# k2-fsa/Flow2GAN

Hardware: AMD Instinct MI355X
Metric: audio-seconds/sec (train step, G+D fwd/bwd) mel_24k_base (higher is better)
Workload: dtype f32 (fp32-class products on the bf16 matrix pipe for the long reductions and the direct MRD convs: every fp32 operand as three bf16 pieces = 24 significand bits, the six v_mfma_f32_32x32x16_bf16 products with i + j <= 2 per fp32 product, fp32 accumulate, error <= 2^-23 per product; short reductions ; 1 GPU; mel_24k_base GAN stage-2 train step: D-step + G-step, each on its own batch (MPD+MRD+FM+multi-scale mel), fwd+bwd+grad all-reduce, no optimizer (metric is fwd/bwd); per_gpu_batch=64, gan=gan_multi_scale_mel_recon, parallelism=dp1, optimizer=none

## Files before the change

flow2gan_amd/csrc/conv2ch.hip:

```cpp
#include <stdlib.h>

#include "common.h"

namespace {

typedef float f32x16 __attribute__((ext_vector_type(16)));

constexpr int KH = 3, KW = 9, NTAP = KH * KW, CO = 32;
constexpr int TW = 32;
constexpr int PW = TW + KW - 1;
constexpr int FTH = 8;
constexpr int FPH = FTH + KH - 1;

__device__ __forceinline__ void stage_patch(float* plane, const f2g_conv2ch_desc& d,
                                            const float* xs, int h0, int w0, int rows, int tid,
                                            int nthreads) {
  for (int i = tid; i < rows * PW; i += nthreads) {
    const int r = i / PW, c = i - r * PW;
    const int h = h0 - 1 + r, w = w0 - 4 + c;
    float2 v = make_float2(0.f, 0.f);
    if (h >= 0 && h < d.H && w >= 0 && w < d.W)
      v = *reinterpret_cast<const float2*>(xs + (long long)h * d.x_line + (long long)w * 2);
    plane[i] = v.x;
    plane[rows * PW + i] = v.y;
  }
}

__global__ __launch_bounds__(256) void conv2ch_fwd_kernel(const f2g_conv2ch_desc d) {
  __shared__ float plane[2 * FPH * PW];
  const int tid = threadIdx.x, lane = tid & 63, wave = tid >> 6;
  const int li = lane & 31, h = lane >> 5;
  const int tiles_w = (d.W + TW - 1) / TW;
  const int tw = blockIdx.x % tiles_w, th = blockIdx.x / tiles_w;
  const int s = blockIdx.y;
  const int h0 = th * FTH, w0 = tw * TW;
  stage_patch(plane, d, d.x + (long long)s * d.x_seq, h0, w0, FPH, tid, 256);
  float bw[NTAP];
#pragma unroll
  for (int t = 0; t < NTAP; ++t) bw[t] = d.w[li * (NTAP * 2) + t * 2 + h];
  const float bias = d.bias ? d.bias[li] : 0.f;
  __syncthreads();
  const float* pl = plane + h * (FPH * PW);
#pragma unroll
  for (int rr = 0; rr < FTH / 4; ++rr) {
    const int row = wave + 4 * rr;
    if (h0 + row >= d.H) break;
    f32x16 acc;
#pragma unroll
    for (int e = 0; e < 16; ++e) acc[e] = bias;
#pragma unroll
    for (int t = 0; t < NTAP; ++t) {
      const int dh = t / KW, j = t - dh * KW;
      const float a = pl[(row + dh) * PW + li + j];
      acc = __builtin_amdgcn_mfma_f32_32x32x2f32(a, bw[t], acc, 0, 0, 0);
    }
    float* yrow = d.y + ((long long)s * d.H + h0 + row) * (long long)d.W * CO;
#pragma unroll
    for (int e = 0; e < 16; ++e) {
      const int col = w0 + (e & 3) + 8 * (e >> 2) + 4 * h;
      if (col < d.W) {
        float v = acc[e];
        if (d.lrelu_slope != 0.f) v = v > 0.f ? v : d.lrelu_slope * v;
        yrow[(long long)col * CO + li] = v;
      }
    }
  }
}

__global__ __launch_bounds__(256) void conv2ch_fwd_p_kernel(const f2g_conv2ch_desc d) {
  __shared__ float plane[2][2 * FPH * PW];
  const int tid = threadIdx.x, lane = tid & 63, wave = tid >> 6;
  const int li = lane & 31, h = lane >> 5;
  const int s = blockIdx.y, w0 = blockIdx.x * TW;
  const float* xs = d.x + (long long)s * d.x_seq;
  float bw[NTAP];
#pragma unroll
  for (int t = 0; t < NTAP; ++t) bw[t] = d.w[li * (NTAP * 2) + t * 2 + h];
  const float bias = d.bias ? d.bias[li] : 0.f;
  constexpr int NP = (FPH * PW + 255) / 256;
  int pr[NP], pc[NP];
#pragma unroll
  for (int q = 0; q < NP; ++q) {
    const int i = tid + 256 * q;
    pr[q] = i / PW;
    pc[q] = i - pr[q] * PW;
  }
  auto load_patch = [&](int h0, float2 (&v)[NP]) {
#pragma unroll
    for (int q = 0; q < NP; ++q) {
      const int hh = h0 - 1 + pr[q], ww = w0 - 4 + pc[q];
      const bool ok = tid + 256 * q < FPH * PW && hh >= 0 && hh < d.H && ww >= 0 && ww < d.W;
      v[q] = ok ? *reinterpret_cast<const float2*>(xs + (long long)hh * d.x_line + (long long)ww * 2)
                : make_float2(0.f, 0.f);
    }
  };
  auto store_patch = [&](float* pl, const float2 (&v)[NP]) {
#pragma unroll
    for (int q = 0; q < NP; ++q) {
      const int i = tid + 256 * q;
      if (i < FPH * PW) {
        pl[i] = v[q].x;
        pl[FPH * PW + i] = v[q].y;
      }
    }
  };
  {
    float2 v[NP];
    load_patch(0, v);
    store_patch(plane[0], v);
  }
  __syncthreads();
  int cur = 0;
  for (int h0 = 0; h0 < d.H; h0 += FTH) {
    const bool more = h0 + FTH < d.H;
    float2 nv[NP];
    load_patch(more ? h0 + FTH : h0, nv);
    const float* pl = plane[cur] + h * (FPH * PW);
#pragma unroll
    for (int rr = 0; rr < FTH / 4; ++rr) {
      const int row = wave + 4 * rr;
      if (h0 + row < d.H) {
        f32x16 acc;
#pragma unroll
        for (int e = 0; e < 16; ++e) acc[e] = bias;
#pragma unroll
        for (int t = 0; t < NTAP; ++t) {
          const int dh = t / KW, j = t - dh * KW;
          acc = __builtin_amdgcn_mfma_f32_32x32x2f32(pl[(row + dh) * PW + li + j], bw[t], acc, 0, 0, 0);
        }
        float* yrow = d.y + ((long long)s * d.H + h0 + row) * (long long)d.W * CO;
#pragma unroll
        for (int e = 0; e < 16; ++e) {
          const int col = w0 + (e & 3) + 8 * (e >> 2) + 4 * h;
          if (col < d.W) {
            float v = acc[e];
            if (d.lrelu_slope != 0.f) v = v > 0.f ? v : d.lrelu_slope * v;
            yrow[(long long)col * CO + li] = v;
          }
        }
      }
    }
    if (more) store_patch(plane[cur ^ 1], nv);
    __syncthreads();
    cur ^= 1;
  }
}

__global__ __launch_bounds__(256) void conv2ch_wgrad_p_kernel(const f2g_conv2ch_desc d, int tiles_h,
                                                              int tiles_w, int tiles_per_block) {
  __shared__ float plane[2 * FPH * PW];
  __shared__ __attribute__((aligned(16))) float gt[FTH * TW * CO];
  const int tid = threadIdx.x, lane = tid & 63, wave = tid >> 6;
  const int li = lane & 31, h = lane >> 5;
  const int ntiles = d.S * tiles_h * tiles_w;
  int boff[2];
  bool bok[2];
#pragma unroll
  for (int nt = 0; nt < 2; ++nt) {
    const int n = li + 32 * nt;
    bok[nt] = n < NTAP * 2;
    const int t = bok[nt] ? n >> 1 : 0, ci = n & 1;
    const int dh = t / KW, j = t - dh * KW;
    boff[nt] = ci * (FPH * PW) + dh * PW + j;
  }
  f32x16 acc[2];
#pragma unroll
  for (int nt = 0; nt < 2; ++nt)
#pragma unroll
    for (int e = 0; e < 16; ++e) acc[nt][e] = 0.f;
  constexpr int NP = (FPH * PW + 255) / 256, NG = FTH * TW * (CO / 4) / 256;
  const int c4 = tid & 7;
  auto load_tile = [&](int ti, float2 (&pv)[NP], float4 (&gv)[NG]) {
    const int s = ti / (tiles_h * tiles_w), rem = ti - s * (tiles_h * tiles_w);
    const int th = rem / tiles_w, tw = rem - th * tiles_w;
    const int h0 = th * FTH, w0 = tw * TW;
    const float* xs = d.x + (long long)s * d.x_seq;
#pragma unroll
    for (int q = 0; q < NP; ++q) {
      const int i = tid + 256 * q, r = i / PW, c = i - r * PW;
      const int hh = h0 - 1 + r, ww = w0 - 4 + c;
      const bool ok = i < FPH * PW && hh >= 0 && hh < d.H && ww >= 0 && ww < d.W;
      pv[q] = ok ? *reinterpret_cast<const float2*>(xs + (long long)hh * d.x_line + (long long)ww * 2)
                 : make_float2(0.f, 0.f);
    }
#pragma unroll
    for (int q = 0; q < NG; ++q) {
      const int px = (tid >> 3) + 32 * q;
      const int row = px / TW, col = px - row * TW;
      const bool ok = h0 + row < d.H && w0 + col < d.W;
      gv[q] = ok ? *reinterpret_cast<const float4*>(d.y + (((long long)s * d.H + h0 + row) * (long long)d.W + w0 + col) * CO + c4 * 4)
                 : make_float4(0.f, 0.f, 0.f, 0.f);
    }
  };
  auto store_tile = [&](const float2 (&pv)[NP], const float4 (&gv)[NG]) {
#pragma unroll
    for (int q = 0; q < NP; ++q) {
      const int i = tid + 256 * q;
      if (i < FPH * PW) {
        plane[i] = pv[q].x;
        plane[FPH * PW + i] = pv[q].y;
      }
    }
#pragma unroll
    for (int q = 0; q < NG; ++q)
      *reinterpret_cast<float4*>(gt + ((tid >> 3) + 32 * q) * CO + c4 * 4) = gv[q];
  };
  const int t0 = blockIdx.x * tiles_per_block;
  int tend = t0 + tiles_per_block;
  if (tend > ntiles) tend = ntiles;
  if (t0 >= tend) return;
  {
    float2 pv[NP];
    float4 gv[NG];
    load_tile(t0, pv, gv);
    store_tile(pv, gv);
  }
  __syncthreads();
  for (int ti = t0; ti < tend; ++ti) {
    const bool more = ti + 1 < tend;
    float2 pv[NP];
    float4 gv[NG];
    load_tile(more ? ti + 1 : ti, pv, gv);
#pragma unroll
    for (int rr = 0; rr < FTH / 4; ++rr) {
      const int row = wave + 4 * rr;
      const float* grow = gt + row * TW * CO + li;
#pragma unroll
      for (int st = 0; st < TW / 2; ++st) {
        const int col = 2 * st + h;
        const float a = grow[col * CO];
        const float b0 = bok[0] ? plane[boff[0] + row * PW + col] : 0.f;
        const float b1 = bok[1] ? plane[boff[1] + row * PW + col] : 0.f;
        acc[0] = __builtin_amdgcn_mfma_f32_32x32x2f32(a, b0, acc[0], 0, 0, 0);
        acc[1] = __builtin_amdgcn_mfma_f32_32x32x2f32(a, b1, acc[1], 0, 0, 0);
      }
    }
    __syncthreads();
    if (more) store_tile(pv, gv);
    __syncthreads();
  }
#pragma unroll
  for (int nt = 0; nt < 2; ++nt) {
    const int n = li + 32 * nt;
    if (n >= NTAP * 2) continue;
#pragma unroll
    for (int e = 0; e < 16; ++e) {
      const int co = (e & 3) + 8 * (e >> 2) + 4 * h;
      atomicAdd(d.gw + co * (NTAP * 2) + n, acc[nt][e]);
    }
  }
}

constexpr int DTH = 8;
constexpr int DPH = DTH + KH - 1;
constexpr int GP = 36;

__global__ __launch_bounds__(256) void conv2ch_dgrad_kernel(const f2g_conv2ch_desc d) {
  extern __shared__ __attribute__((aligned(16))) float gp[];
  const int tid = threadIdx.x;
  const int tiles_w = (d.W + TW - 1) / TW;
  const int tw = blockIdx.x % tiles_w, th = blockIdx.x / tiles_w;
  const int s = blockIdx.y;
  const int h0 = th * DTH, w0 = tw * TW;
  const float* gs = d.y + (long long)s * d.H * d.W * CO;
  for (int i = tid; i < DPH * PW * (CO / 4); i += 256) {
    const int c4 = i & 7, px = i >> 3;
    const int r = px / PW, c = px - r * PW;
    const int hh = h0 - 1 + r, ww = w0 - 4 + c;
    float4 v = make_float4(0.f, 0.f, 0.f, 0.f);
    if (hh >= 0 && hh < d.H && ww >= 0 && ww < d.W)
      v = *reinterpret_cast<const float4*>(gs + ((long long)hh * d.W + ww) * CO + c4 * 4);
    *reinterpret_cast<float4*>(gp + px * GP + c4 * 4) = v;
  }
  __syncthreads();
  const int pw = tid & 31, ph = tid >> 5;
  float a0 = 0.f, a1 = 0.f;
#pragma unroll
  for (int dh = 0; dh < KH; ++dh)
#pragma unroll
    for (int j = 0; j < KW; ++j) {
      const float* g0 = gp + ((ph + 2 - dh) * PW + pw + 8 - j) * GP;
      const float* wt = d.wt + (dh * KW + j) * (2 * CO);
#pragma unroll
      for (int c4 = 0; c4 < CO / 4; ++c4) {
        const float4 gv = *reinterpret_cast<const float4*>(g0 + c4 * 4);
        a0 += gv.x * wt[c4 * 4] + gv.y * wt[c4 * 4 + 1] + gv.z * wt[c4 * 4 + 2] + gv.w * wt[c4 * 4 + 3];
        a1 += gv.x * wt[CO + c4 * 4] + gv.y * wt[CO + c4 * 4 + 1] + gv.z * wt[CO + c4 * 4 + 2] +
              gv.w * wt[CO + c4 * 4 + 3];
      }
    }
  const int hh = h0 + ph, ww = w0 + pw;
  if (hh < d.H && ww < d.W) {
    float* o = d.gx + (long long)s * d.gx_seq + (long long)hh * d.gx_line + (long long)ww * 2;
    *reinterpret_cast<float2*>(o) = make_float2(a0, a1);
  }
}

constexpr int QTH = 8, QTW = 32;
constexpr int QPH = QTH + 2, QPW = QTW + 2;

__device__ __forceinline__ void stage32(float* patch, const float* xs, int H, int W, int h0, int w0,
                                        int tid) {
  for (int i = tid; i < QPH * QPW * (CO / 4); i += 256) {
    const int c4 = i & 7, px = i >> 3;
    const int r = px / QPW, c = px - r * QPW;
    const int hh = h0 - 1 + r, ww = w0 - 1 + c;
    float4 v = make_float4(0.f, 0.f, 0.f, 0.f);
    if (hh >= 0 && hh < H && ww >= 0 && ww < W)
      v = *reinterpret_cast<const float4*>(xs + ((long long)hh * W + ww) * CO + c4 * 4);
    *reinterpret_cast<float4*>(patch + px * GP + c4 * 4) = v;
  }
}

__global__ __launch_bounds__(256) void convpost_fwd_kernel(const f2g_conv2ch_desc d) {
  extern __shared__ __attribute__((aligned(16))) float patch[];
  const int tid = threadIdx.x;
  const int tiles_w = (d.W + QTW - 1) / QTW;
  const int tw = blockIdx.x % tiles_w, th = blockIdx.x / tiles_w;
  const int s = blockIdx.y;
  const int h0 = th * QTH, w0 = tw * QTW;
  __shared__ __attribute__((aligned(16))) float wl[9 * CO];
  for (int i = tid; i < 9 * CO; i += 256) wl[i] = d.w[i];
  stage32(patch, d.x + (long long)s * d.H * d.W * CO, d.H, d.W, h0, w0, tid);
  __syncthreads();
  const int pw = tid & 31, ph = tid >> 5;
  float a0 = 0.f, a1 = 0.f;
#pragma unroll 1
  for (int t = 0; t < 9; ++t) {
    const float* x0 = patch + ((ph + t / 3) * QPW + pw + t % 3) * GP;
    const float* wt = wl + t * CO;
#pragma unroll
    for (int c4 = 0; c4 < CO / 4; c4 += 2) {
      const float4 u = *reinterpret_cast<const float4*>(x0 + c4 * 4);
      const float4 v = *reinterpret_cast<const float4*>(x0 + c4 * 4 + 4);
      const float4 wu = *reinterpret_cast<const float4*>(wt + c4 * 4);
      const float4 wv = *reinterpret_cast<const float4*>(wt + c4 * 4 + 4);
      a0 += u.x * wu.x + u.y * wu.y + u.z * wu.z + u.w * wu.w;
      a1 += v.x * wv.x + v.y * wv.y + v.z * wv.z + v.w * wv.w;
    }
  }
  const int hh = h0 + ph, ww = w0 + pw;
  if (hh < d.H && ww < d.W)
    d.y[((long long)s * d.H + hh) * d.W + ww] = a0 + a1 + (d.bias ? d.bias[0] : 0.f);
}

__global__ __launch_bounds__(256) void convpost_wgrad_kernel(const f2g_conv2ch_desc d, int px_per_block) {
  __shared__ float red[32][9 * CO + 1];
  const int tid = threadIdx.x, c4 = tid & 7, pg = tid >> 3;
  const long long npx = (long long)d.S * d.H * d.W;
  float4 acc[9];
#pragma unroll
  for (int t = 0; t < 9; ++t) acc[t] = make_float4(0.f, 0.f, 0.f, 0.f);
  const long long p0 = (long long)blockIdx.x * px_per_block;
  const long long pend = p0 + px_per_block < npx ? p0 + px_per_block : npx;
  constexpr int U = 4;
  for (long long p = p0 + pg; p < pend; p += 32 * U) {
    float4 v[U];
    float gn[U][9];
#pragma unroll
    for (int u = 0; u < U; ++u) {
      const long long q = p + 32 * u;
      const bool on = q < pend;
      const long long qq = on ? q : p;
      v[u] = *reinterpret_cast<const float4*>(d.x + qq * CO + c4 * 4);
      const int w = (int)(qq % d.W);
      const int h = (int)((qq / d.W) % d.H);
#pragma unroll
      for (int t = 0; t < 9; ++t) {
        const int oh = h - (t / 3 - 1), ow = w - (t % 3 - 1);
        const bool ok = on && oh >= 0 && oh < d.H && ow >= 0 && ow < d.W;
        gn[u][t] = ok ? d.y[qq - (long long)(t / 3 - 1) * d.W - (t % 3 - 1)] : 0.f;
      }
    }
#pragma unroll
    for (int u = 0; u < U; ++u)
#pragma unroll
      for (int t = 0; t < 9; ++t) {
        acc[t].x += gn[u][t] * v[u].x; acc[t].y += gn[u][t] * v[u].y;
        acc[t].z += gn[u][t] * v[u].z; acc[t].w += gn[u][t] * v[u].w;
      }
  }
#pragma unroll
  for (int t = 0; t < 9; ++t) {
    red[pg][t * CO + c4 * 4 + 0] = acc[t].x; red[pg][t * CO + c4 * 4 + 1] = acc[t].y;
    red[pg][t * CO + c4 * 4 + 2] = acc[t].z; red[pg][t * CO + c4 * 4 + 3] = acc[t].w;
  }
  __syncthreads();
  for (int k = tid; k < 9 * CO; k += 256) {
    float s = 0.f;
#pragma unroll 8
    for (int g2 = 0; g2 < 32; ++g2) s += red[g2][k];
    atomicAdd(d.gw + k, s);
  }
}

__global__ __launch_bounds__(256) void convpost_dgrad_kernel(const f2g_conv2ch_desc d) {
  const long long npx = (long long)d.S * d.H * d.W;
  const int c4 = threadIdx.x & 7;
  float4 wv[9];
#pragma unroll
  for (int t = 0; t < 9; ++t) wv[t] = *reinterpret_cast<const float4*>(d.w + t * CO + c4 * 4);
  for (long long i = (long long)blockIdx.x * 32 + (threadIdx.x >> 3); i < npx;
       i += (long long)gridDim.x * 32) {
    const int ww = (int)(i % d.W);
    const long long q = i / d.W;
    const int hh = (int)(q % d.H);
    float4 a = make_float4(0.f, 0.f, 0.f, 0.f);
#pragma unroll
    for (int t = 0; t < 9; ++t) {
      const int sh = hh + 1 - t / 3, sw = ww + 1 - t % 3;
      if (sh >= 0 && sh < d.H && sw >= 0 && sw < d.W) {
        const float gv = d.y[i + (long long)(1 - t / 3) * d.W + (1 - t % 3)];
        a.x += gv * wv[t].x; a.y += gv * wv[t].y; a.z += gv * wv[t].z; a.w += gv * wv[t].w;
      }
    }
    *reinterpret_cast<float4*>(d.gx + i * CO + c4 * 4) = a;
  }
}

}

#define ST ((hipStream_t)stream)

static bool conv2ch_ok(const f2g_conv2ch_desc* d) {
  return d && d->S > 0 && d->H > 0 && d->W > 0;
}

extern "C" int f2g_conv2ch_fwd(const f2g_conv2ch_desc* d, f2g_stream_t stream) {
  if (!d || !d->x || !d->w || !d->y || (d->x_line & 1) || (d->x_seq & 1)) return F2G_EINVAL;
  if (!conv2ch_ok(d)) return F2G_OK;
  if ((long long)((d->W + TW - 1) / TW) * d->S >= 256) {
    hipLaunchKernelGGL(conv2ch_fwd_p_kernel, dim3((d->W + TW - 1) / TW, d->S), dim3(256), 0, ST, *d);
    return f2g_check_launch();
  }
  const int tiles = ((d->H + FTH - 1) / FTH) * ((d->W + TW - 1) / TW);
  hipLaunchKernelGGL(conv2ch_fwd_kernel, dim3(tiles, d->S), dim3(256), 0, ST, *d);
  return f2g_check_launch();
}

extern "C" int f2g_conv2ch_wgrad(const f2g_conv2ch_desc* d, f2g_stream_t stream) {
  if (!d || !d->x || !d->y || !d->gw || (d->x_line & 1) || (d->x_seq & 1)) return F2G_EINVAL;
  if (((uintptr_t)d->y) & 15) return F2G_EINVAL;
  if (!conv2ch_ok(d)) return F2G_OK;
  const int tiles_h = (d->H + FTH - 1) / FTH, tiles_w = (d->W + TW - 1) / TW;
  const int ntiles = d->S * tiles_h * tiles_w;
  int per = (ntiles + 511) / 512;
  if (per < 1) per = 1;
  hipLaunchKernelGGL(conv2ch_wgrad_p_kernel, dim3((ntiles + per - 1) / per), dim3(256), 0, ST, *d,
                     tiles_h, tiles_w, per);
  return f2g_check_launch();
}

extern "C" int f2g_conv2ch_dgrad(const f2g_conv2ch_desc* d, f2g_stream_t stream) {
  if (!d || !d->y || !d->wt || !d->gx || (d->gx_line & 1) || (d->gx_seq & 1)) return F2G_EINVAL;
  if ((((uintptr_t)d->y) & 15) || (((uintptr_t)d->gx) & 7)) return F2G_EINVAL;
  if (!conv2ch_ok(d)) return F2G_OK;
  const size_t smem = (size_t)DPH * PW * GP * sizeof(float);
  static bool attr_done = false;
  if (!attr_done) {
    (void)hipFuncSetAttribute(reinterpret_cast<const void*>(conv2ch_dgrad_kernel),
                              hipFuncAttributeMaxDynamicSharedMemorySize, (int)smem);
    attr_done = true;
  }
  const int tiles = ((d->H + DTH - 1) / DTH) * ((d->W + TW - 1) / TW);
  hipLaunchKernelGGL(conv2ch_dgrad_kernel, dim3(tiles, d->S), dim3(256), smem, ST, *d);
  return f2g_check_launch();
}

extern "C" int f2g_convpost_fwd(const f2g_conv2ch_desc* d, f2g_stream_t stream) {
  if (!d || !d->x || !d->w || !d->y || (((uintptr_t)d->x) & 15)) return F2G_EINVAL;
  if (!conv2ch_ok(d)) return F2G_OK;
  const size_t smem = (size_t)QPH * QPW * GP * sizeof(float);
  static bool attr_done = false;
  if (!attr_done) {
    (void)hipFuncSetAttribute(reinterpret_cast<const void*>(convpost_fwd_kernel),
                              hipFuncAttributeMaxDynamicSharedMemorySize, (int)smem);
    attr_done = true;
  }
  const int tiles = ((d->H + QTH - 1) / QTH) * ((d->W + QTW - 1) / QTW);
  hipLaunchKernelGGL(convpost_fwd_kernel, dim3(tiles, d->S), dim3(256), smem, ST, *d);
  return f2g_check_launch();
}

extern "C" int f2g_convpost_wgrad(const f2g_conv2ch_desc* d, f2g_stream_t stream) {
  if (!d || !d->x || !d->y || !d->gw || (((uintptr_t)d->x) & 15)) return F2G_EINVAL;
  if (!conv2ch_ok(d)) return F2G_OK;
  const long long npx = (long long)d->S * d->H * d->W;
  long long per = (npx + 1023) / 1024;
  if (per < 128) per = 128;
  hipLaunchKernelGGL(convpost_wgrad_kernel, dim3((unsigned)((npx + per - 1) / per)), dim3(256), 0, ST, *d, (int)per);
  return f2g_check_launch();
}

extern "C" int f2g_convpost_dgrad(const f2g_conv2ch_desc* d, f2g_stream_t stream) {
  if (!d || !d->y || !d->w || !d->gx || (((uintptr_t)d->gx) & 15) || (((uintptr_t)d->w) & 15))
    return F2G_EINVAL;
  if (!conv2ch_ok(d)) return F2G_OK;
  const long long npx = (long long)d->S * d->H * d->W;
  hipLaunchKernelGGL(convpost_dgrad_kernel, dim3(f2g_grid_for(npx, 32, 16384)), dim3(256), 0, ST, *d);
  return f2g_check_launch();
}
```

Measured before the change: 794.9 audio-s/s.

## Restructure 2-channel MRD conv fwd/wgrad into flattened pixel chunks with LDS reduction

The forward and weight-gradient kernels for the 2-input-channel 3x9 conv now walk flattened pixel chunks of 512 over column segments instead of fixed 8x32 tiles. This keeps MFMA lanes fully busy for narrow or short spectrogram shapes. The forward swaps the MFMA operand roles so each lane writes float4-vectorized outputs. Wgrad precomputes pixel offsets in LDS, double-buffers gradient loads, and reduces per block in LDS before global atomics. The dgrad inner loop is rewritten as a software-pipelined f32x4 FMA sequence with scalar-memory weights and explicit waitcnt/sched barriers. Costs are larger dynamic shared memory, extra index indirection, and hand-tuned scheduling that is fragile across compilers.

```diff
diff --git a/flow2gan_amd/csrc/conv2ch.hip b/flow2gan_amd/csrc/conv2ch.hip
--- a/flow2gan_amd/csrc/conv2ch.hip
+++ b/flow2gan_amd/csrc/conv2ch.hip
@@ -4,239 +4,168 @@
 
 namespace {
 
+typedef float f32x4 __attribute__((ext_vector_type(4)));
 typedef float f32x16 __attribute__((ext_vector_type(16)));
 
 constexpr int KH = 3, KW = 9, NTAP = KH * KW, CO = 32;
-constexpr int TW = 32;
-constexpr int PW = TW + KW - 1;
-constexpr int FTH = 8;
-constexpr int FPH = FTH + KH - 1;
-
-__device__ __forceinline__ void stage_patch(float* plane, const f2g_conv2ch_desc& d,
-                                            const float* xs, int h0, int w0, int rows, int tid,
-                                            int nthreads) {
-  for (int i = tid; i < rows * PW; i += nthreads) {
-    const int r = i / PW, c = i - r * PW;
-    const int h = h0 - 1 + r, w = w0 - 4 + c;
+constexpr int PXB = 512;
+constexpr int WSEG = 1024;
+
+__host__ __device__ inline int chunk_rows(int H, int Wc) {
+  const int n = (PXB - 1) / Wc + 4;
+  return n < H + 2 ? n : H + 2;
+}
+
+__device__ __forceinline__ void stage_rows(float* plane, int ps, const f2g_conv2ch_desc& d, const float* xs,
+                                           int c0, int Wc, int r0, int nrows, int tid) {
+  const int pw = Wc + KW - 1, n = nrows * pw;
+#pragma unroll 4
+  for (int i = tid; i < n; i += 256) {
+    const int r = i / pw, c = i - r * pw;
+    const int hh = r0 - 1 + r, ww = c0 - 4 + c;
     float2 v = make_float2(0.f, 0.f);
-    if (h >= 0 && h < d.H && w >= 0 && w < d.W)
-      v = *reinterpret_cast<const float2*>(xs + (long long)h * d.x_line + (long long)w * 2);
+    if (hh >= 0 && hh < d.H && ww >= 0 && ww < d.W)
+      v = *reinterpret_cast<const float2*>(xs + (long long)hh * d.x_line + (long long)ww * 2);
     plane[i] = v.x;
-    plane[rows * PW + i] = v.y;
-  }
-}
-
-__global__ __launch_bounds__(256) void conv2ch_fwd_kernel(const f2g_conv2ch_desc d) {
-  __shared__ float plane[2 * FPH * PW];
+    plane[ps + i] = v.y;
+  }
+}
+
+__global__ __launch_bounds__(256) void conv2ch_fwd_kernel(const f2g_conv2ch_desc d, int c0, int Wc,
+                                                          int chunks_per_seq, int chunks_per_block) {
+  extern __shared__ float planes[];
   const int tid = threadIdx.x, lane = tid & 63, wave = tid >> 6;
   const int li = lane & 31, h = lane >> 5;
-  const int tiles_w = (d.W + TW - 1) / TW;
-  const int tw = blockIdx.x % tiles_w, th = blockIdx.x / tiles_w;
-  const int s = blockIdx.y;
-  const int h0 = th * FTH, w0 = tw * TW;
-  stage_patch(plane, d, d.x + (long long)s * d.x_seq, h0, w0, FPH, tid, 256);
-  float bw[NTAP];
-#pragma unroll
-  for (int t = 0; t < NTAP; ++t) bw[t] = d.w[li * (NTAP * 2) + t * 2 + h];
-  const float bias = d.bias ? d.bias[li] : 0.f;
-  __syncthreads();
-  const float* pl = plane + h * (FPH * PW);
-#pragma unroll
-  for (int rr = 0; rr < FTH / 4; ++rr) {
-    const int row = wave + 4 * rr;
-    if (h0 + row >= d.H) break;
-    f32x16 acc;
-#pragma unroll
-    for (int e = 0; e < 16; ++e) acc[e] = bias;
-#pragma unroll
-    for (int t = 0; t < NTAP; ++t) {
-      const int dh = t / KW, j = t - dh * KW;
-      const float a = pl[(row + dh) * PW + li + j];
-      acc = __builtin_amdgcn_mfma_f32_32x32x2f32(a, bw[t], acc, 0, 0, 0);
-    }
-    float* yrow = d.y + ((long long)s * d.H + h0 + row) * (long long)d.W * CO;
-#pragma unroll
-    for (int e = 0; e < 16; ++e) {
-      const int col = w0 + (e & 3) + 8 * (e >> 2) + 4 * h;
-      if (col < d.W) {
-        float v = acc[e];
-        if (d.lrelu_slope != 0.f) v = v > 0.f ? v : d.lrelu_slope * v;
-        yrow[(long long)col * CO + li] = v;
-      }
-    }
-  }
-}
-
-__global__ __launch_bounds__(256) void conv2ch_fwd_p_kernel(const f2g_conv2ch_desc d) {
-  __shared__ float plane[2][2 * FPH * PW];
+  const int npx = d.H * Wc, pw = Wc + KW - 1, ps = chunk_rows(d.H, Wc) * pw;
+  const int nchunks = d.S * chunks_per_seq;
+  const int k0 = blockIdx.x * chunks_per_block;
+  const int k1 = k0 + chunks_per_block < nchunks ? k0 + chunks_per_block : nchunks;
+  if (k0 >= k1) return;
+  auto stage_chunk = [&](int k, float* buf) {
+    const int s = k / chunks_per_seq, p0 = (k - s * chunks_per_seq) * PXB;
+    const int p1 = p0 + PXB < npx ? p0 + PXB : npx;
+    const int r0 = p0 / Wc, r1 = (p1 - 1) / Wc;
+    stage_rows(buf, ps, d, d.x + (long long)s * d.x_seq, c0, Wc, r0, r1 - r0 + 3, tid);
+  };
+  stage_chunk(k0, planes);
+  float aw[NTAP];
+#pragma unroll
+  for (int t = 0; t < NTAP; ++t) aw[t] = d.w[li * (NTAP * 2) + t * 2 + h];
+  f32x16 bias;
+#pragma unroll
+  for (int e = 0; e < 16; ++e) bias[e] = d.bias ? d.bias[8 * (e >> 2) + 4 * h + (e & 3)] : 0.f;
+  __syncthreads();
+  for (int k = k0; k < k1; ++k) {
+    const int cur = (k - k0) & 1;
+    if (k + 1 < k1) stage_chunk(k + 1, planes + (cur ^ 1) * 2 * ps);
+    const int s = k / chunks_per_seq, p0 = (k - s * chunks_per_seq) * PXB;
+    const int p1 = p0 + PXB < npx ? p0 + PXB : npx;
+    const int r0 = p0 / Wc;
+    const float* pl = planes + cur * 2 * ps + h * ps;
+    for (int g0 = p0 + wave * 32; g0 < p1; g0 += 128) {
+      const int p = g0 + li, pp = p < p1 ? p : p1 - 1;
+      const int r = pp / Wc, c = pp - r * Wc;
+      const float* q = pl + (r - r0) * pw + c;
+      f32x16 acc = bias;
+#pragma unroll
+      for (int t = 0; t < NTAP; ++t) {
+        const int dh = t / KW, j = t - dh * KW;
+        acc = __builtin_amdgcn_mfma_f32_32x32x2f32(aw[t], q[dh * pw + j], acc, 0, 0, 0);
+      }
+      if (p < p1) {
+        float* o = d.y + (((long long)s * d.H + r) * d.W + c0 + c) * CO + 4 * h;
+#pragma unroll
+        for (int e4 = 0; e4 < 4; ++e4) {
+          f32x4 v = {acc[4 * e4], acc[4 * e4 + 1], acc[4 * e4 + 2], acc[4 * e4 + 3]};
+          if (d.lrelu_slope != 0.f) {
+#pragma unroll
+            for (int i = 0; i < 4; ++i) v[i] = v[i] > 0.f ? v[i] : d.lrelu_slope * v[i];
+          }
+          *reinterpret_cast<f32x4*>(o + 8 * e4) = v;
+        }
+      }
+    }
+    __syncthreads();
+  }
+}
+
+__global__ __launch_bounds__(256) void conv2ch_wgrad_kernel(const f2g_conv2ch_desc d, int c0, int Wc,
+                                                            int chunks_per_seq, int chunks_per_block) {
+  extern __shared__ float sm[];
   const int tid = threadIdx.x, lane = tid & 63, wave = tid >> 6;
   const int li = lane & 31, h = lane >> 5;
-  const int s = blockIdx.y, w0 = blockIdx.x * TW;
-  const float* xs = d.x + (long long)s * d.x_seq;
-  float bw[NTAP];
-#pragma unroll
-  for (int t = 0; t < NTAP; ++t) bw[t] = d.w[li * (NTAP * 2) + t * 2 + h];
-  const float bias = d.bias ? d.bias[li] : 0.f;
-  constexpr int NP = (FPH * PW + 255) / 256;
-  int pr[NP], pc[NP];
-#pragma unroll
-  for (int q = 0; q < NP; ++q) {
-    const int i = tid + 256 * q;
-    pr[q] = i / PW;
-    pc[q] = i - pr[q] * PW;
-  }
-  auto load_patch = [&](int h0, float2 (&v)[NP]) {
-#pragma unroll
-    for (int q = 0; q < NP; ++q) {
-      const int hh = h0 - 1 + pr[q], ww = w0 - 4 + pc[q];
-      const bool ok = tid + 256 * q < FPH * PW && hh >= 0 && hh < d.H && ww >= 0 && ww < d.W;
-      v[q] = ok ? *reinterpret_cast<const float2*>(xs + (long long)hh * d.x_line + (long long)ww * 2)
-                : make_float2(0.f, 0.f);
-    }
-  };
-  auto store_patch = [&](float* pl, const float2 (&v)[NP]) {
-#pragma unroll
-    for (int q = 0; q < NP; ++q) {
-      const int i = tid + 256 * q;
-      if (i < FPH * PW) {
-        pl[i] = v[q].x;
-        pl[FPH * PW + i] = v[q].y;
-      }
-    }
-  };
-  {
-    float2 v[NP];
-    load_patch(0, v);
-    store_patch(plane[0], v);
-  }
-  __syncthreads();
-  int cur = 0;
-  for (int h0 = 0; h0 < d.H; h0 += FTH) {
-    const bool more = h0 + FTH < d.H;
-    float2 nv[NP];
-    load_patch(more ? h0 + FTH : h0, nv);
-    const float* pl = plane[cur] + h * (FPH * PW);
-#pragma unroll
-    for (int rr = 0; rr < FTH / 4; ++rr) {
-      const int row = wave + 4 * rr;
-      if (h0 + row < d.H) {
-        f32x16 acc;
-#pragma unroll
-        for (int e = 0; e < 16; ++e) acc[e] = bias;
-#pragma unroll
-        for (int t = 0; t < NTAP; ++t) {
-          const int dh = t / KW, j = t - dh * KW;
-          acc = __builtin_amdgcn_mfma_f32_32x32x2f32(pl[(row + dh) * PW + li + j], bw[t], acc, 0, 0, 0);
-        }
-        float* yrow = d.y + ((long long)s * d.H + h0 + row) * (long long)d.W * CO;
-#pragma unroll
-        for (int e = 0; e < 16; ++e) {
-          const int col = w0 + (e & 3) + 8 * (e >> 2) + 4 * h;
-          if (col < d.W) {
-            float v = acc[e];
-            if (d.lrelu_slope != 0.f) v = v > 0.f ? v : d.lrelu_slope * v;
-            yrow[(long long)col * CO + li] = v;
-          }
-        }
-      }
-    }
-    if (more) store_patch(plane[cur ^ 1], nv);
-    __syncthreads();
-    cur ^= 1;
-  }
-}
-
-__global__ __launch_bounds__(256) void conv2ch_wgrad_p_kernel(const f2g_conv2ch_desc d, int tiles_h,
-                                                              int tiles_w, int tiles_per_block) {
-  __shared__ float plane[2 * FPH * PW];
-  __shared__ __attribute__((aligned(16))) float gt[FTH * TW * CO];
-  const int tid = threadIdx.x, lane = tid & 63, wave = tid >> 6;
-  const int li = lane & 31, h = lane >> 5;
-  const int ntiles = d.S * tiles_h * tiles_w;
+  const int npx = d.H * Wc, pw = Wc + KW - 1, ps = chunk_rows(d.H, Wc) * pw;
+  const int bufsz = 2 * ps + 2 * PXB;
+  float* red = sm;
+  float* bufs = sm + CO * NTAP * 2;
+  const int nchunks = d.S * chunks_per_seq;
+  const int k0 = blockIdx.x * chunks_per_block;
+  const int k1 = k0 + chunks_per_block < nchunks ? k0 + chunks_per_block : nchunks;
+  if (k0 >= k1) return;
+  for (int i = tid; i < CO * NTAP * 2; i += 256) red[i] = 0.f;
   int boff[2];
-  bool bok[2];
 #pragma unroll
   for (int nt = 0; nt < 2; ++nt) {
     const int n = li + 32 * nt;
-    bok[nt] = n < NTAP * 2;
-    const int t = bok[nt] ? n >> 1 : 0, ci = n & 1;
+    const int t = n < NTAP * 2 ? n >> 1 : 0, ci = n & 1;
     const int dh = t / KW, j = t - dh * KW;
-    boff[nt] = ci * (FPH * PW) + dh * PW + j;
+    boff[nt] = ci * ps + dh * pw + j;
   }
   f32x16 acc[2];
 #pragma unroll
   for (int nt = 0; nt < 2; ++nt)
 #pragma unroll
     for (int e = 0; e < 16; ++e) acc[nt][e] = 0.f;
-  constexpr int NP = (FPH * PW + 255) / 256, NG = FTH * TW * (CO / 4) / 256;
-  const int c4 = tid & 7;
-  auto load_tile = [&](int ti, float2 (&pv)[NP], float4 (&gv)[NG]) {
-    const int s = ti / (tiles_h * tiles_w), rem = ti - s * (tiles_h * tiles_w);
-    const int th = rem / tiles_w, tw = rem - th * tiles_w;
-    const int h0 = th * FTH, w0 = tw * TW;
-    const float* xs = d.x + (long long)s * d.x_seq;
-#pragma unroll
-    for (int q = 0; q < NP; ++q) {
-      const int i = tid + 256 * q, r = i / PW, c = i - r * PW;
-      const int hh = h0 - 1 + r, ww = w0 - 4 + c;
-      const bool ok = i < FPH * PW && hh >= 0 && hh < d.H && ww >= 0 && ww < d.W;
-      pv[q] = ok ? *reinterpret_cast<const float2*>(xs + (long long)hh * d.x_line + (long long)ww * 2)
-                 : make_float2(0.f, 0.f);
-    }
-#pragma unroll
-    for (int q = 0; q < NG; ++q) {
-      const int px = (tid >> 3) + 32 * q;
-      const int row = px / TW, col = px - row * TW;
-      const bool ok = h0 + row < d.H && w0 + col < d.W;
-      gv[q] = ok ? *reinterpret_cast<const float4*>(d.y + (((long long)s * d.H + h0 + row) * (long long)d.W + w0 + col) * CO + c4 * 4)
-                 : make_float4(0.f, 0.f, 0.f, 0.f);
+  auto stage_chunk = [&](int k, float* buf) {
+    const int s = k / chunks_per_seq, p0 = (k - s * chunks_per_seq) * PXB;
+    const int p1 = p0 + PXB < npx ? p0 + PXB : npx;
+    const int r0 = p0 / Wc, r1 = (p1 - 1) / Wc;
+    stage_rows(buf, ps, d, d.x + (long long)s * d.x_seq, c0, Wc, r0, r1 - r0 + 3, tid);
+    int* tpos = reinterpret_cast<int*>(buf + 2 * ps);
+    for (int i = tid; i < PXB; i += 256) {
+      const int p = p0 + i;
+      const bool ok = p < p1;
+      const int r = ok ? p / Wc : r0, c = ok ? p - r * Wc : 0;
+      tpos[i] = (r - r0) * pw + c;
+      tpos[PXB + i] = r * d.W + c;
     }
   };
-  auto store_tile = [&](const float2 (&pv)[NP], const float4 (&gv)[NG]) {
-#pragma unroll
-    for (int q = 0; q < NP; ++q) {
-      const int i = tid + 256 * q;
-      if (i < FPH * PW) {
-        plane[i] = pv[q].x;
-        plane[FPH * PW + i] = pv[q].y;
-      }
-    }
-#pragma unroll
-    for (int q = 0; q < NG; ++q)
-      *reinterpret_cast<float4*>(gt + ((tid >> 3) + 32 * q) * CO + c4 * 4) = gv[q];
-  };
-  const int t0 = blockIdx.x * tiles_per_block;
-  int tend = t0 + tiles_per_block;
-  if (tend > ntiles) tend = ntiles;
-  if (t0 >= tend) return;
-  {
-    float2 pv[NP];
-    float4 gv[NG];
-    load_tile(t0, pv, gv);
-    store_tile(pv, gv);
-  }
-  __syncthreads();
-  for (int ti = t0; ti < tend; ++ti) {
-    const bool more = ti + 1 < tend;
-    float2 pv[NP];
-    float4 gv[NG];
-    load_tile(more ? ti + 1 : ti, pv, gv);
-#pragma unroll
-    for (int rr = 0; rr < FTH / 4; ++rr) {
-      const int row = wave + 4 * rr;
-      const float* grow = gt + row * TW * CO + li;
-#pragma unroll
-      for (int st = 0; st < TW / 2; ++st) {
-        const int col = 2 * st + h;
-        const float a = grow[col * CO];
-        const float b0 = bok[0] ? plane[boff[0] + row * PW + col] : 0.f;
-        const float b1 = bok[1] ? plane[boff[1] + row * PW + col] : 0.f;
-        acc[0] = __builtin_amdgcn_mfma_f32_32x32x2f32(a, b0, acc[0], 0, 0, 0);
-        acc[1] = __builtin_amdgcn_mfma_f32_32x32x2f32(a, b1, acc[1], 0, 0, 0);
-      }
-    }
-    __syncthreads();
-    if (more) store_tile(pv, gv);
+  stage_chunk(k0, bufs);
+  __syncthreads();
+  for (int k = k0; k < k1; ++k) {
+    const int cur = (k - k0) & 1;
+    if (k + 1 < k1) stage_chunk(k + 1, bufs + (cur ^ 1) * bufsz);
+    const int s = k / chunks_per_seq, p0 = (k - s * chunks_per_seq) * PXB;
+    const int cnt = (p0 + PXB < npx ? p0 + PXB : npx) - p0;
+    const float* pl = bufs + cur * bufsz;
+    const int* tpos = reinterpret_cast<const int*>(pl + 2 * ps);
+    const float* gs = d.y + ((long long)s * d.H * d.W + c0) * CO + li;
+    auto load_group = [&](int g0, float (&a)[16]) {
+#pragma unroll
+      for (int st = 0; st < 16; ++st) {
+        const int i = g0 + 2 * st + h;
+        const float v = gs[(long long)tpos[PXB + i] * CO];
+        a[st] = i < cnt ? v : 0.f;
+      }
+    };
+    float a[16];
+    int g0 = wave * 32;
+    if (g0 < cnt) load_group(g0, a);
+    for (; g0 < cnt; g0 += 128) {
+      float an[16];
+      const bool more = g0 + 128 < cnt;
+      if (more) load_group(g0 + 128, an);
+#pragma unroll
+      for (int st = 0; st < 16; ++st) {
+        const int pos = tpos[g0 + 2 * st + h];
+        acc[0] = __builtin_amdgcn_mfma_f32_32x32x2f32(a[st], pl[boff[0] + pos], acc[0], 0, 0, 0);
+        acc[1] = __builtin_amdgcn_mfma_f32_32x32x2f32(a[st], pl[boff[1] + pos], acc[1], 0, 0, 0);
+      }
+      if (more) {
+#pragma unroll
+        for (int st = 0; st < 16; ++st) a[st] = an[st];
+      }
+    }
     __syncthreads();
   }
 #pragma unroll
@@ -246,11 +175,15 @@
 #pragma unroll
     for (int e = 0; e < 16; ++e) {
       const int co = (e & 3) + 8 * (e >> 2) + 4 * h;
-      atomicAdd(d.gw + co * (NTAP * 2) + n, acc[nt][e]);
-    }
-  }
-}
-
+      atomicAdd(red + co * (NTAP * 2) + n, acc[nt][e]);
+    }
+  }
+  __syncthreads();
+  for (int i = tid; i < CO * NTAP * 2; i += 256) atomicAdd(d.gw + i, red[i]);
+}
+
+constexpr int TW = 32;
+constexpr int PW = TW + KW - 1;
 constexpr int DTH = 8;
 constexpr int DPH = DTH + KH - 1;
 constexpr int GP = 36;
@@ -274,25 +207,49 @@
   }
   __syncthreads();
   const int pw = tid & 31, ph = tid >> 5;
-  float a0 = 0.f, a1 = 0.f;
-#pragma unroll
-  for (int dh = 0; dh < KH; ++dh)
-#pragma unroll
-    for (int j = 0; j < KW; ++j) {
-      const float* g0 = gp + ((ph + 2 - dh) * PW + pw + 8 - j) * GP;
-      const float* wt = d.wt + (dh * KW + j) * (2 * CO);
-#pragma unroll
-      for (int c4 = 0; c4 < CO / 4; ++c4) {
-        const float4 gv = *reinterpret_cast<const float4*>(g0 + c4 * 4);
-        a0 += gv.x * wt[c4 * 4] + gv.y * wt[c4 * 4 + 1] + gv.z * wt[c4 * 4 + 2] + gv.w * wt[c4 * 4 + 3];
-        a1 += gv.x * wt[CO + c4 * 4] + gv.y * wt[CO + c4 * 4 + 1] + gv.z * wt[CO + c4 * 4 + 2] +
-              gv.w * wt[CO + c4 * 4 + 3];
-      }
-    }
+  f32x4 a0 = {0.f, 0.f, 0.f, 0.f}, a1 = {0.f, 0.f, 0.f, 0.f};
+  typedef __attribute__((address_space(4))) float cfloat;
+  constexpr int NST = NTAP * 2;
+  struct stage { f32x4 g[4], w0[4], w1[4]; };
+  const float* gbase = gp + ((ph + 2) * PW + pw + 8) * GP;
+  auto load_stage = [&](int st, stage& b) {
+    const int t = st >> 1, half = st & 1;
+    const int dh = t / KW, j = t - dh * KW;
+    const float* g0 = gbase - (dh * PW + j) * GP + half * 16;
+    const cfloat* wt = (const cfloat*)(d.wt) + t * (2 * CO) + half * 16;
+#pragma unroll
+    for (int q = 0; q < 4; ++q) {
+      b.g[q] = *reinterpret_cast<const f32x4*>(g0 + q * 4);
+      b.w0[q] = f32x4{wt[q * 4], wt[q * 4 + 1], wt[q * 4 + 2], wt[q * 4 + 3]};
+      b.w1[q] = f32x4{wt[CO + q * 4], wt[CO + q * 4 + 1], wt[CO + q * 4 + 2], wt[CO + q * 4 + 3]};
+    }
+  };
+  auto fma_stage = [&](const stage& b) {
+#pragma unroll
+    for (int q = 0; q < 4; ++q) {
+      a0 += b.g[q] * b.w0[q];
+      a1 += b.g[q] * b.w1[q];
+    }
+  };
+  stage sa, sb;
+  load_stage(0, sa);
+#pragma unroll 1
+  for (int st = 0; st < NST; st += 2) {
+    __builtin_amdgcn_s_waitcnt(0xc07f);
+    load_stage(st + 1, sb);
+    __builtin_amdgcn_sched_barrier(0);
+    fma_stage(sa);
+    __builtin_amdgcn_sched_barrier(0);
+    __builtin_amdgcn_s_waitcnt(0xc07f);
+    load_stage(st + 2 < NST ? st + 2 : st, sa);
+    __builtin_amdgcn_sched_barrier(0);
+    fma_stage(sb);
+    __builtin_amdgcn_sched_barrier(0);
+  }
   const int hh = h0 + ph, ww = w0 + pw;
   if (hh < d.H && ww < d.W) {
     float* o = d.gx + (long long)s * d.gx_seq + (long long)hh * d.gx_line + (long long)ww * 2;
-    *reinterpret_cast<float2*>(o) = make_float2(a0, a1);
+    *reinterpret_cast<float2*>(o) = make_float2((a0[0] + a0[1]) + (a0[2] + a0[3]), (a1[0] + a1[1]) + (a1[2] + a1[3]));
   }
 }
 
@@ -426,29 +383,55 @@
   return d && d->S > 0 && d->H > 0 && d->W > 0;
 }
 
+constexpr int kMaxChunkSmem = 96 * 1024;
+
 extern "C" int f2g_conv2ch_fwd(const f2g_conv2ch_desc* d, f2g_stream_t stream) {
   if (!d || !d->x || !d->w || !d->y || (d->x_line & 1) || (d->x_seq & 1)) return F2G_EINVAL;
-  if (!conv2ch_ok(d)) return F2G_OK;
-  if ((long long)((d->W + TW - 1) / TW) * d->S >= 256) {
-    hipLaunchKernelGGL(conv2ch_fwd_p_kernel, dim3((d->W + TW - 1) / TW, d->S), dim3(256), 0, ST, *d);
-    return f2g_check_launch();
-  }
-  const int tiles = ((d->H + FTH - 1) / FTH) * ((d->W + TW - 1) / TW);
-  hipLaunchKernelGGL(conv2ch_fwd_kernel, dim3(tiles, d->S), dim3(256), 0, ST, *d);
-  return f2g_check_launch();
+  if (((uintptr_t)d->y) & 15) return F2G_EINVAL;
+  if (!conv2ch_ok(d)) return F2G_OK;
+  static bool attr_done = false;
+  if (!attr_done) {
+    (void)hipFuncSetAttribute(reinterpret_cast<const void*>(conv2ch_fwd_kernel),
+                              hipFuncAttributeMaxDynamicSharedMemorySize, kMaxChunkSmem);
+    attr_done = true;
+  }
+  for (int c0 = 0; c0 < d->W; c0 += WSEG) {
+    const int Wc = d->W - c0 < WSEG ? d->W - c0 : WSEG;
+    const int per_seq = (d->H * Wc + PXB - 1) / PXB;
+    const long long nchunks = (long long)d->S * per_seq;
+    const long long per = (nchunks + 1279) / 1280;
+    const size_t smem = (size_t)4 * chunk_rows(d->H, Wc) * (Wc + KW - 1) * sizeof(float);
+    hipLaunchKernelGGL(conv2ch_fwd_kernel, dim3((unsigned)((nchunks + per - 1) / per)), dim3(256), smem, ST, *d,
+                       c0, Wc, per_seq, (int)per);
+    const int rc = f2g_check_launch();
+    if (rc != F2G_OK) return rc;
+  }
+  return F2G_OK;
 }
 
 extern "C" int f2g_conv2ch_wgrad(const f2g_conv2ch_desc* d, f2g_stream_t stream) {
   if (!d || !d->x || !d->y || !d->gw || (d->x_line & 1) || (d->x_seq & 1)) return F2G_EINVAL;
   if (((uintptr_t)d->y) & 15) return F2G_EINVAL;
   if (!conv2ch_ok(d)) return F2G_OK;
-  const int tiles_h = (d->H + FTH - 1) / FTH, tiles_w = (d->W + TW - 1) / TW;
-  const int ntiles = d->S * tiles_h * tiles_w;
-  int per = (ntiles + 511) / 512;
-  if (per < 1) per = 1;
-  hipLaunchKernelGGL(conv2ch_wgrad_p_kernel, dim3((ntiles + per - 1) / per), dim3(256), 0, ST, *d,
-                     tiles_h, tiles_w, per);
-  return f2g_check_launch();
+  static bool attr_done = false;
+  if (!attr_done) {
+    (void)hipFuncSetAttribute(reinterpret_cast<const void*>(conv2ch_wgrad_kernel),
+                              hipFuncAttributeMaxDynamicSharedMemorySize, kMaxChunkSmem);
+    attr_done = true;
+  }
+  for (int c0 = 0; c0 < d->W; c0 += WSEG) {
+    const int Wc = d->W - c0 < WSEG ? d->W - c0 : WSEG;
+    const int per_seq = (d->H * Wc + PXB - 1) / PXB;
+    const long long nchunks = (long long)d->S * per_seq;
+    const long long per = (nchunks + 1023) / 1024;
+    const size_t smem = ((size_t)CO * NTAP * 2 + (size_t)2 * (2 * chunk_rows(d->H, Wc) * (Wc + KW - 1) + 2 * PXB)) *
+                        sizeof(float);
+    hipLaunchKernelGGL(conv2ch_wgrad_kernel, dim3((unsigned)((nchunks + per - 1) / per)), dim3(256), smem, ST, *d,
+                       c0, Wc, per_seq, (int)per);
+    const int rc = f2g_check_launch();
+    if (rc != F2G_OK) return rc;
+  }
+  return F2G_OK;
 }
 
 extern "C" int f2g_conv2ch_dgrad(const f2g_conv2ch_desc* d, f2g_stream_t stream) {
```

Result: no change. 793.5 audio-s/s (-0.2%).
